# facebookresearch/momentum

Hardware: NVIDIA H100
Metric: GN iterations/sec (batched 72-joint IK) (higher is better)
Workload: dtype f32

## Files before the change

### include/momentum_b200.h

```cpp
#ifndef MOMENTUM_B200_H_
#define MOMENTUM_B200_H_

#include <stddef.h>
#include <stdint.h>

#ifdef __cplusplus
extern "C" {
#endif

#define MB2_PARAMETERS_PER_JOINT 7
#define MB2_MAX_MODEL_PARAMETERS 2048
#define MB2_PARAMETER_SET_WORDS 32

typedef enum mb2_status {
  MB2_OK = 0,
  MB2_ERR_INVALID_ARGUMENT = 1,
  MB2_ERR_CUDA = 2,
  MB2_ERR_UNSUPPORTED = 3
} mb2_status;

typedef enum mb2_instance_status {
  MB2_INSTANCE_OK = 0,
  MB2_INSTANCE_CHOLESKY_BREAKDOWN = 1,
  MB2_INSTANCE_NON_FINITE = 2
// ... 242 lines not shown
int mb2_solver_function_implicit_direction_device(mb2_solver_function* f, const float* parameters_device ,
                                                  const float* grad_parameters_device , float* direction_device ,
                                                  float* jacobian_direction_device , float* residual_device ,
                                                  float* gradient_rms_device , void* cuda_stream);

int mb2_solver_create(mb2_solver_function* f, const mb2_gauss_newton_options* opt, mb2_solver** out);
void mb2_solver_destroy(mb2_solver* s);
int mb2_solver_set_options(mb2_solver* s, const mb2_gauss_newton_options* opt);
int mb2_solver_set_enabled_parameters(mb2_solver* s, const uint64_t bits[MB2_PARAMETER_SET_WORDS]);
int mb2_solver_solve(mb2_solver* s, float* parameters, double* errors, int32_t* iterations, int32_t* status);
int mb2_solver_solve_async(mb2_solver* s, float* parameters);
int mb2_solver_wait(mb2_solver* s, double* errors, int32_t* iterations, int32_t* status);
int mb2_solver_solve_device(mb2_solver* s, float* parameters_device, void* cuda_stream);
int mb2_solver_get_results(mb2_solver* s, double* errors, int32_t* iterations, int32_t* status);
int mb2_solver_get_error_history(mb2_solver* s, double* history);
int mb2_solver_get_counters(mb2_solver* s, uint64_t* total_iterations, uint64_t* kernel_launches);
int mb2_solver_set_profiling(mb2_solver* s, int32_t enabled);
int mb2_solver_get_phase_times(mb2_solver* s, double ms[4], uint64_t launches[4]);
int mb2_solver_get_plan_stats(mb2_solver* s, int64_t stats[12]);
int mb2_solver_get_fused_profile(mb2_solver* s, int32_t* fused, int32_t* groups, double* kernel_ms, uint64_t phase_cycles[12]);
int mb2_solver_function_get_sweep_launch(mb2_solver_function* f, int32_t jacobian, int64_t out[5]);
int mb2_character_get_instance_launch(const mb2_character* c, int32_t op, int32_t backward, int32_t batch, int32_t num_points, int64_t out[6]);
int mb2_solver_function_get_input_gradient_launch(mb2_solver_function* f, int64_t out[6]);
int mb2_solver_get_solve_path(mb2_solver* s, int64_t out[15]);

typedef struct mb2_mixed_batch mb2_mixed_batch;
const char* mb2_mixed_batch_last_error(void);
int mb2_mixed_batch_create(int device, int32_t granule , mb2_mixed_batch** out);
void mb2_mixed_batch_destroy(mb2_mixed_batch* b);
int mb2_mixed_batch_add_rig(mb2_mixed_batch* b, const mb2_character* c, int32_t num_parameters, int32_t* rig_id);
int mb2_mixed_batch_use_limits(mb2_mixed_batch* b, int32_t enabled, float weight);
int mb2_mixed_batch_add_instance(mb2_mixed_batch* b, int32_t rig_id, int32_t num_constraints, const int32_t* parents, const float* offsets ,
                                 const float* weights , const float* targets , const float* theta0 , int32_t* instance_id);
int mb2_mixed_batch_set_parameters(mb2_mixed_batch* b, int32_t instance_id, const float* theta0);
int mb2_mixed_batch_solve(mb2_mixed_batch* b, const mb2_gauss_newton_options* opt);
int mb2_mixed_batch_get_result(mb2_mixed_batch* b, int32_t instance_id, float* theta, double* error, int32_t* iterations, int32_t* status);
int mb2_mixed_batch_get_results(mb2_mixed_batch* b, float* theta, const int64_t* theta_offsets, double* errors, int32_t* iterations, int32_t* status);
int mb2_mixed_batch_stats(mb2_mixed_batch* b, int64_t stats[6]);
int mb2_mixed_batch_bucket_info(mb2_mixed_batch* b, int32_t bucket, int64_t info[4]);

int mb2_character_clone(const mb2_character* c, int device, mb2_character** out);
int mb2_solver_function_clone(const mb2_solver_function* f, const mb2_character* c_on_device, int32_t batch, mb2_solver_function** out);
int mb2_character_device(const mb2_character* c);
const mb2_character* mb2_solver_function_character(const mb2_solver_function* f);
int32_t mb2_solver_function_num_error_functions(const mb2_solver_function* f);
int32_t mb2_solver_function_target_size(const mb2_solver_function* f, int32_t index);

// ... 17 lines not shown
```

### momentum_b200/csrc/ik_capi.cu

```cuda
#include "../../include/momentum_b200.h"

#include <cuda_runtime.h>
#include <nvtx3/nvToolsExt.h>

#include <algorithm>
#include <cfloat>
#include <cmath>
#include <cstdio>
#include <cstdlib>
#include <cstring>
#include <memory>
#include <string>
#include <vector>

#include "ik_chol_sched.h"
#include "ik_fused.cuh"
#include "ik_jtj_tc.cuh"
#include "ik_kernels.cuh"
#include "ik_plan.h"
#include "ik_solve_path.h"

using namespace mb2;

namespace {
// ... 163 lines not shown
  std::unique_ptr<DeviceSchedule> sched;
  SweepLaunch lastSweep[2]{};
  FunctionTables tables() const;
};

struct PhaseEvent {
  cudaEvent_t start, stop;
  int phase;
};

struct mb2_solver {
  mb2_solver_function* fn{nullptr};
  mb2_gauss_newton_options opt{};
  DeviceBuffer<float> dH, dDelta, dThetaOrig, dTheta0, dScale, dGradDotDelta, dThetaStage, dGrad, dTiles, dRadius, dRSaved;
  DeviceBuffer<double> dLastErrors, dTrialErrors, dHistory;
  DeviceBuffer<int32_t> dActive, dIterations, dStatus, dSearching, dActiveCount, dWorkCounter, dQrChunks;
  DeviceBuffer<unsigned long long> dPhaseCycles;
  DeviceBuffer<float> dPark;
  DeviceBuffer<uint32_t> dParkSlots;
  SolvePath path;
  cudaEvent_t fusedStart{nullptr}, fusedStop{nullptr};
  double fusedMs{0};
  int* hActiveCount{nullptr};
  char* hResults{nullptr};
  size_t hResultsBytes{0};
  bool resultsStaged{false};
  uint64_t totalIterations{0}, kernelLaunches{0};
  bool profiling{false};
  bool inKernelProfile{false};
  std::vector<PhaseEvent> events;
  double phaseMs[4]{0, 0, 0, 0};
  uint64_t phaseLaunches[4]{0, 0, 0, 0};
  size_t historyStride{0};
  ~mb2_solver() {
    if (hActiveCount) cudaFreeHost(hActiveCount);
    if (hResults) cudaFreeHost(hResults);
    if (fusedStart) cudaEventDestroy(fusedStart);
    if (fusedStop) cudaEventDestroy(fusedStop);
    for (auto& e : events) { cudaEventDestroy(e.start); cudaEventDestroy(e.stop); }
  }
};

CharacterTables mb2_character::tables() const {
  CharacterTables C{};
  C.numJoints = host.numJoints;
  C.numParams = host.numParams;
  C.parent = parent.p;
  C.offset = offset.p;
  C.prerot = prerot.p;
  C.ptOuter = ptOuter.p;
  C.ptInner = ptInner.p;
  C.ptVals = ptVals.p;
  C.ptOffsets = ptOffsets.p;
  C.numLevels = int(host.levelStart.size()) - 1;
  C.ptNnz = int(host.ptInner.size());
  C.levelStart = levelStart.p;
  C.levelJoints = levelJoints.p;
  return C;
}

SkeletonTables mb2_character::skeletonTables() const {
  return SkeletonTables{childStart.p, children.p,  ptColStart.p, ptColRows.p, ptColVals.p, invStart.p,
// ... 1406 lines not shown
  a.enabledList = f->dEnabledList.p;
  a.numEnabled = int(f->plan.enabledList.size());
  a.gradParameters = grad_parameters_device;
  a.direction = direction_device;
  a.jacobianDirection = jacobian_direction_device;
  a.residual = residual_device;
  a.gradientRms = gradient_rms_device;
  ImplicitDirectionConfig cfg;
  MB2_CUDA(implicitDirectionConfigure(a, cfg));
  MB2_CUDA(f->dJacobi.resize(std::max<size_t>(1, size_t(cfg.grid) * cfg.slotDoubles)));
  a.scratch = f->dJacobi.p;
  a.slotDoubles = cfg.slotDoubles;
  a.gramInShared = cfg.gramInShared ? 1 : 0;
  MB2_CUDA(launchImplicitDirection(a, cfg, st));
  return MB2_OK;
}

int mb2_solver_create(mb2_solver_function* f, const mb2_gauss_newton_options* opt, mb2_solver** out) {
  MB2_CHECK(f != nullptr && out != nullptr, "null argument");
  auto s = std::make_unique<mb2_solver>();
  s->fn = f;
  if (opt) s->opt = *opt; else mb2_default_gauss_newton_options(&s->opt);
  MB2_DEVICE_GUARD(f->ch->device);
  MB2_CUDA(cudaMallocHost(&s->hActiveCount, sizeof(int)));
  *out = s.release();
  return MB2_OK;
}
void mb2_solver_destroy(mb2_solver* s) { delete s; }
int mb2_solver_set_options(mb2_solver* s, const mb2_gauss_newton_options* opt) {
  MB2_CHECK(s != nullptr && opt != nullptr, "null argument");
  s->opt = *opt;
  return MB2_OK;
}
int mb2_solver_set_enabled_parameters(mb2_solver* s, const uint64_t* bits) {
  MB2_CHECK(s != nullptr, "null solver");
  return mb2_solver_function_set_enabled_parameters(s->fn, bits);
}
int mb2_solver_set_profiling(mb2_solver* s, int32_t enabled) {
  MB2_CHECK(s != nullptr, "null solver");
  s->profiling = enabled != 0;
  s->inKernelProfile = enabled >= 2;
  return MB2_OK;
}

namespace {
int planFigures(mb2_solver_function* f, int mode, bool schedDense, bool strips, PlanFigures& F, std::string& msg) {
  const int rc = ensurePlan(f, mode, schedDense, strips);
// ... 12 lines not shown
    F.gramCholValid = ds->gcValid;
    F.fusedBlobWords = ds->fLayout.words;
  }
  return MB2_OK;
}

}

int mb2_solver_solve_device(mb2_solver* s, float* theta, void* cudaStream) {
  MB2_CHECK(s != nullptr && theta != nullptr, "null argument");
  mb2_solver_function* f = s->fn;
  MB2_DEVICE_GUARD(f->ch->device);
  NvtxRange nvtxSolve("mb2::SolverT::solve");
  const mb2_gauss_newton_options& o = s->opt;
  const DeviceLimits lim = deviceLimits();
  std::string msg;
  const PlanFiguresFn plan = [f](int mode, bool schedDense, bool strips, PlanFigures& F, std::string& m) { return planFigures(f, mode, schedDense, strips, F, m); };
  int rc = chooseSolvePath(o, f->B, f->ch->host, f->host, plan, lim, s->path, msg);
  if (s->path.planMode != 0 && f->sched) f->sched->fusedGroups = s->path.fused.groups;
  if (rc != MB2_OK) {
    s->path = SolvePath{};
    return fail(rc, msg);
  }
  const SolvePath& P = s->path;
  cudaStream_t st = cudaStream ? (cudaStream_t)cudaStream : f->stream;
  const int B = f->B, n = f->ch->host.numParams;
  const int ns = f->plan.numCols;
  const int maxIt = int(std::min<uint64_t>(o.max_iterations, 1u << 30));
  const int minIt = int(std::min<uint64_t>(o.min_iterations, 1u << 30));
  MB2_CUDA(s->dIterations.resize(B));
  MB2_CUDA(s->dStatus.resize(B));
  if (o.store_error_history) {
    MB2_CUDA(s->dHistory.resize(size_t(B) * std::max(maxIt, 1)));
    MB2_CUDA(cudaMemsetAsync(s->dHistory.p, 0, size_t(B) * std::max(maxIt, 1) * sizeof(double), st));
    s->historyStride = size_t(std::max(maxIt, 1));
  }
  for (auto& e : s->events) { cudaEventDestroy(e.start); cudaEventDestroy(e.stop); }
  s->events.clear();
  if (s->profiling && (P.kind == kSolvePersistent || P.kind == kSolveGramCholesky)) {
    MB2_CUDA(s->dPhaseCycles.resize(16));
    MB2_CUDA(cudaMemsetAsync(s->dPhaseCycles.p, 0, 16 * sizeof(unsigned long long), st));
  }
  if (P.kind == kSolvePersistent) {
    const DeviceSchedule& ds = *f->sched;
    MB2_CUDA(s->dWorkCounter.resize(1));
    MB2_CUDA(cudaMemsetAsync(s->dWorkCounter.p, 0, sizeof(int32_t), st));
// ... 32 lines not shown
      MB2_CUDA(launchFusedSolve(fa, P.fused, lim.numSms, s->inKernelProfile, st));
    }
    if (s->profiling) MB2_CUDA(cudaEventRecord(s->fusedStop, st));
    s->kernelLaunches = 1;
    return MB2_OK;
  }
  const int ldH = roundUp(ns + 1, 16);
  const size_t hStride = size_t(ns + 1) * ldH;
  if (P.kind == kSolveDense || P.kind == kSolveTilesKMajor) MB2_CUDA(s->dH.resize(size_t(B) * hStride));
  const size_t tilesStride = P.strips ? size_t(f->sched->host.numTiles) * 256 + f->sched->host.nPad : 0;
  if (P.kind == kSolveTiles) MB2_CUDA(s->dTiles.resize(size_t(B) * tilesStride));
  const bool qr = P.kind == kSolveQr || P.kind == kSolveTrustRegionQr;
  if (qr) MB2_CUDA(s->dQrChunks.upload(P.qrChunkStarts, st));
  if (P.kind == kSolveTrustRegionQr) {
    MB2_CUDA(s->dRadius.upload(std::vector<float>(size_t(B), o.trust_region_radius), st));
    MB2_CUDA(s->dRSaved.resize(size_t(B) * P.trRSavedFloats));
  }
  const int ldG = cholGradientLd(ns);
  MB2_CUDA(s->dGrad.resize(size_t(B) * ldG));
  MB2_CUDA(s->dDelta.resize(size_t(B) * ns));
  MB2_CUDA(s->dTheta0.resize(size_t(B) * n));
  MB2_CUDA(s->dLastErrors.resize(B));
  MB2_CUDA(s->dActive.resize(B));
  MB2_CUDA(s->dActiveCount.resize(1));
  const bool lineSearch = o.do_line_search != 0 && P.kind != kSolveTrustRegionQr;
  if (lineSearch) {
    MB2_CUDA(s->dThetaOrig.resize(size_t(B) * n));
    MB2_CUDA(s->dTrialErrors.resize(B));
    MB2_CUDA(s->dScale.resize(B));
    MB2_CUDA(s->dSearching.resize(B));
    MB2_CUDA(s->dGradDotDelta.resize(B));
  }
  double* history = o.store_error_history ? s->dHistory.p : nullptr;

  const SweepArgs sweep = sweepArgs(f, theta, s->dActive.p);
  GramArgs g{};
  if (P.strips) {
    const DeviceSchedule& ds = *f->sched;
    g.batch = B;
    g.strips = f->dJ.p;
    g.stripStride = size_t(ds.gram.stride);
    g.residOff = ds.gram.residOff;
    g.active = s->dActive.p;
    g.numStrips = ds.gram.numStrips;
    g.numTiles = ds.host.numTiles;
    g.numTileCols = ds.host.numTileCols;
    g.nPad = ds.host.nPad;
// ... 74 lines not shown
    }
    gt.L = ds.gc.L;
    gt.tab = ds.gcTab.p;
  }
  CholArgs& step = qr ? t.q.c : (P.kind == kSolveGramCholesky ? gc.c : c);
  SweepArgs trial = sweepArgs(f, theta, s->dSearching.p);
  trial.errors = s->dTrialErrors.p;
  LineSearchArgs la{};
  la.batch = B; la.ns = ns; la.numParams = n; la.ldTheta = n;
  la.errors = f->dErrors.p;
  la.trialErrors = s->dTrialErrors.p;
  la.gradDotDelta = s->dGradDotDelta.p;
  la.scale = s->dScale.p;
  la.searching = s->dSearching.p;
  la.subsetVariant = o.subset_line_search;
  la.active = s->dActive.p;
  BookkeepingArgs ba{};
  ba.batch = B;
  ba.errors = f->dErrors.p; ba.lastErrors = s->dLastErrors.p; ba.active = s->dActive.p; ba.iterations = s->dIterations.p;
  ba.status = s->dStatus.p; ba.history = history;
  ba.theta = theta; ba.ldTheta = n; ba.numParams = n;
  ba.minIterations = minIt; ba.maxIterations = maxIt; ba.threshold = o.threshold; ba.activeCount = s->dActiveCount.p;

  s->kernelLaunches = 0;
  initSolveStateKernel<<<(B + 127) / 128, 128, 0, st>>>(B, s->dActive.p, s->dIterations.p, s->dStatus.p, s->dLastErrors.p, f->dErrors.p);
  MB2_CUDA(cudaGetLastError());
  MB2_CUDA(cudaMemcpyAsync(s->dTheta0.p, theta, size_t(B) * n * sizeof(float), cudaMemcpyDeviceToDevice, st));

  static const bool cholProfile = getenv("MB2_CHOL_PROFILE") != nullptr;
  constexpr int kPollEvery = 4;
  for (int it = 0; it < maxIt; ++it) {
    MB2_CUDA(cudaMemsetAsync(s->dActiveCount.p, 0, sizeof(int), st));
    recordPhaseStart(s, 0, st);
    MB2_CUDA(launchSweep(sweep, true, st, &f->lastSweep[1]));
    recordPhaseStop(s, st);
    step.iteration = it;
    step.profile = (it == 0 && cholProfile) ? 1 : 0;
    switch (P.kind) {
      case kSolveDense:
      case kSolveTilesKMajor:
      case kSolveTiles:
        recordPhaseStart(s, 1, st);
        if (P.kind == kSolveTiles) MB2_CUDA(launchGramTiles(g, P.gramThreads, st));
        else if ((rc = runJtJ(f, P.jtjMode, ns, c.H, ldH, hStride, s->dActive.p, st, s->dGrad.p, ldG)) != MB2_OK) return rc;
        recordPhaseStop(s, st);
        recordPhaseStart(s, 2, st);
        if (P.kind == kSolveDense) MB2_CUDA(launchCholesky(c, P.denseNb, P.denseInSmem, st));
        else MB2_CUDA(launchCholeskyScheduled(c, f->sched->dev, P.cholThreads, st));
        break;
      case kSolveGramCholesky:
        recordPhaseStart(s, 2, st);
        MB2_CUDA(launchGramCholesky(gc, f->sched->dev, f->sched->gcParams.get(), gt, s->inKernelProfile, st));
        break;
      case kSolveQr:
        recordPhaseStart(s, 2, st);
        MB2_CUDA(launchQrSolve(t.q, P.qrWidestChunk, st));
        break;
      default:
        recordPhaseStart(s, 2, st);
        MB2_CUDA(launchTrustRegionQr(t, st));
    }
    recordPhaseStop(s, st);
    if (lineSearch) {
      MB2_CUDA(cudaMemcpyAsync(s->dThetaOrig.p, theta, size_t(B) * n * sizeof(float), cudaMemcpyDeviceToDevice, st));
      initLineSearchKernel<<<(B + 127) / 128, 128, 0, st>>>(B, s->dActive.p, s->dSearching.p, s->dScale.p);
      MB2_CUDA(cudaGetLastError());
      for (int k = 0; k < 10; ++k) {
        MB2_CUDA(launchTrialUpdate(B, s->dThetaOrig.p, n, s->dDelta.p, ns, f->dDeviceCols.p, s->dScale.p, theta, s->dSearching.p, st));
        recordPhaseStart(s, 3, st);
        MB2_CUDA(launchSweep(trial, false, st, &f->lastSweep[0]));
        recordPhaseStop(s, st);
        la.step = k;
        MB2_CUDA(launchLineSearchStep(la, st));
        s->kernelLaunches += 2;
      }
      ba.iteration = it;
      MB2_CUDA(launchBookkeeping(ba, st));
      s->kernelLaunches += 1;
    }
    if (it + 1 < maxIt && it >= minIt && (it - minIt) % kPollEvery == kPollEvery - 1) {
      MB2_CUDA(cudaMemcpyAsync(s->hActiveCount, s->dActiveCount.p, sizeof(int), cudaMemcpyDeviceToHost, st));
      MB2_CUDA(cudaStreamSynchronize(st));
      if (*s->hActiveCount == 0) break;
    }
  }
  finalizeKernel<<<B, 128, 0, st>>>(B, n, theta, s->dTheta0.p, s->dStatus.p);
  MB2_CUDA(cudaGetLastError());
  s->kernelLaunches += 2;
  return MB2_OK;
}

static void collectProfile(mb2_solver* s) {
  if (s->profiling && s->path.kind == kSolvePersistent && s->fusedStart) {
    float ms = 0.f;
    s->fusedMs = cudaEventElapsedTime(&ms, s->fusedStart, s->fusedStop) == cudaSuccess ? double(ms) : 0.0;
  }
  if (s->profiling) {
    for (int k = 0; k < 4; ++k) { s->phaseMs[k] = 0; s->phaseLaunches[k] = 0; }
    for (auto& e : s->events) {
      float ms = 0.f;
      if (cudaEventElapsedTime(&ms, e.start, e.stop) == cudaSuccess) { s->phaseMs[e.phase] += ms; s->phaseLaunches[e.phase]++; }
    }
  }
}

int mb2_solver_get_results(mb2_solver* s, double* errors, int32_t* iterations, int32_t* status) {
  MB2_CHECK(s != nullptr, "null solver");
  mb2_solver_function* f = s->fn;
// ... 177 lines not shown
    a.T = c->tables();
    a.numChildren = int(c->host.children.size());
    a.batch = batch;
    a.P.numPoints = num_points;
    a.fromJointParameters = joint;
    MB2_CUDA(queryPositionsLaunch(a, backward != 0, &q));
  }
  instanceLaunchWords(q, out);
  return MB2_OK;
}

int mb2_solver_function_get_input_gradient_launch(mb2_solver_function* f, int64_t out[6]) {
  MB2_CHECK(f != nullptr && out != nullptr, "null argument");
  MB2_DEVICE_GUARD(f->ch->device);
  InputGradientArgs a{};
  a.T = f->tables();
  a.batch = f->B;
  InstanceLaunchQuery q;
  MB2_CUDA(launchInputGradients(a, nullptr, &q));
  instanceLaunchWords(q, out);
  return MB2_OK;
}

int mb2_solver_get_solve_path(mb2_solver* s, int64_t out[15]) {
  MB2_CHECK(s != nullptr && out != nullptr, "null argument");
  solvePathWords(s->path, out);
  return MB2_OK;
}

int mb2_solver_get_phase_times(mb2_solver* s, double ms[4], uint64_t launches[4]) {
  MB2_CHECK(s != nullptr, "null solver");
  for (int k = 0; k < 4; ++k) {
    if (ms) ms[k] = s->phaseMs[k];
    if (launches) launches[k] = s->phaseLaunches[k];
  }
  return MB2_OK;
}

}
```

### momentum_b200/csrc/ik_kernels.cu

```cuda
#include "ik_kernels.cuh"

#include <algorithm>
#include <cstdio>
#include <type_traits>

#include "ik_chol.cuh"
#include "ik_chol_sched.h"
#include "ik_jtj_tc.cuh"
#include "ik_ptx.cuh"
#include "ik_device.cuh"
#include "ik_jacobi.cuh"

namespace mb2 {

__device__ __forceinline__ double warpSum(double v) {
  for (int o = 16; o > 0; o >>= 1) v += __shfl_xor_sync(0xffffffffu, v, o);
  return v;
}

size_t sweepSmemPerInstance(const FunctionTables& T, int warpsPerInstance) {
  const size_t nPad = (T.numParams + 3) & ~3;
  const size_t jp = warpsPerInstance > 1 ? size_t((T.numJoints * kParametersPerJoint + 1) & ~1) : 0;
  return sizeof(float) * (nPad + jp + size_t((T.numJoints * kJointStateStride + 1) & ~1) + size_t((T.recStride + 1) & ~1) + 4 + 2 * size_t(warpsPerInstance));
}
// ... 69 lines not shown
    }
    g.sync();
  }
}

static int g_numSms = 0;
static int g_maxSmemOptin = 0;
static int g_maxSmemPerSm = 0;

cudaError_t launchSweep(const SweepArgs& a0, bool jacobian, cudaStream_t stream, SweepLaunch* out) {
  SweepArgs a = a0;
  if (out) *out = SweepLaunch{};
  const size_t budget = size_t(g_maxSmemOptin);
  const size_t per1 = sweepSmemPerInstance(a.T, 8);
  a.stageTables = (2 * per1 + sweepTableBytes(a.T, 1) + 16 <= budget) ? 1 : (2 * per1 + sweepTableBytes(a.T, 2) + 16 <= budget) ? 2 : 0;
  const size_t tableBytes = sweepTableBytes(a.T, a.stageTables) + 16;
  int groups = int((budget - tableBytes) / per1);
  if (groups < 1) return cudaErrorInvalidConfiguration;
  const int groupsOneWarp = int((budget - tableBytes) / sweepSmemPerInstance(a.T, 1));
  int W = 1;
  if (groupsOneWarp >= 16) {
    const int sms = std::max(g_numSms, 1);
    const int maxG = std::min(groupsOneWarp, kSweepMaxWarps), minG = std::min(12, maxG);
    long best = -1;
    if (a.batch < sms * minG) { groups = std::max(1, (a.batch + sms - 1) / sms); best = 0; }
    for (int gcand = maxG; gcand >= minG && best != 0; --gcand) {
      const long rounds = (a.batch + long(sms) * gcand - 1) / (long(sms) * gcand);
      if (best < 0 || rounds * gcand < best) { best = rounds * gcand; groups = gcand; }
    }
  } else {
    if (groups > 15) groups = 15;
    while (W < 8 && groups * W * 2 <= kSweepMaxWarps) W *= 2;
  }
  a.warpsPerInstance = W;
  const int warps = groups * W;
  const size_t per = sweepSmemPerInstance(a.T, W);
  const size_t smem = per * groups + tableBytes;
  if (smem > budget) return cudaErrorInvalidConfiguration;
  const int ctasNeeded = (a.batch + groups - 1) / groups;
  int ctasPerSm = (int)((size_t(g_maxSmemPerSm)) / (smem + 1024));
  if (ctasPerSm < 1) ctasPerSm = 1;
  if (ctasPerSm * warps > 32) ctasPerSm = 32 / warps > 0 ? 32 / warps : 1;
  int grid = g_numSms * ctasPerSm;
  if (grid > ctasNeeded) grid = ctasNeeded;
  if (grid < 1) grid = 1;
  if (out) *out = SweepLaunch{a.stageTables, W, groups, grid, int64_t(smem)};
  auto launch = [&](auto kernel) -> cudaError_t {
    const cudaError_t e = cudaFuncSetAttribute(kernel, cudaFuncAttributeMaxDynamicSharedMemorySize, int(smem));
    if (e != cudaSuccess) return e;
    kernel<<<grid, warps * 32, smem, stream>>>(a);
// ... 1903 lines not shown
  const uint64_t strides[2] = {uint64_t(fromGram ? 256 : a.ldH) * sizeof(float), uint64_t(fromGram ? a.tilesStride : a.hStride) * sizeof(float)};
  const uint32_t box[3] = {16u, 16u, 1u};
  e = makeTensorMap3d(&hmap, fromGram ? a.tilesIn : a.H, dims, strides, box, 64);
  if (e != cudaSuccess) return e;
  if (wide && prof) choleskyScheduledKernel<512, true><<<a.batch, 512, smem, stream>>>(hmap, a, sched);
  else if (wide) choleskyScheduledKernel<512, false><<<a.batch, 512, smem, stream>>>(hmap, a, sched);
  else if (prof) choleskyScheduledKernel<256, true><<<a.batch, 256, smem, stream>>>(hmap, a, sched);
  else choleskyScheduledKernel<256, false><<<a.batch, 256, smem, stream>>>(hmap, a, sched);
  return cudaGetLastError();
}

__device__ int acquireParkSlot(uint32_t* words, int numWords, int start) {
  for (int w = start % numWords;; w = (w + 1 == numWords) ? 0 : w + 1) {
    uint32_t freeBits = ~__ldcg(words + w);
    while (freeBits != 0u) {
      const int bit = __ffs(freeBits) - 1;
      if ((atomicOr(words + w, 1u << bit) & (1u << bit)) == 0u) return 32 * w + bit;
      freeBits &= freeBits - 1u;
    }
  }
}

template <bool kProfile, class Tables>
__global__ void __launch_bounds__(kGramThreads, 4) gramCholeskyKernel(const GramCholArgs a, const CholSchedDev S, const __grid_constant__ Tables P) {
  extern __shared__ __align__(16) float gcSmem[];
  const GramArgs& g = a.g;
  const CholArgs& c = a.c;
  const int b = blockIdx.x;
  if (c.active[b] == 0) return;
  const int n = c.ns, tid = threadIdx.x;
  const int warp = tid >> 5, lane = tid & 31, hw = tid >> 4, hl = tid & 15;
  constexpr int kWarps = kGramThreads / 32;
  float* U = gcSmem + (((128u - (smemAddr(gcSmem) & 127u)) & 127u) >> 2);
  const size_t tileFloats = size_t(S.numTiles) * 256, sweepFloats = g.stripStride + 64;
  const size_t uni = ((tileFloats > sweepFloats ? tileFloats : sweepFloats) + 3) & ~size_t(3);
  float* strips = U;
  float* resid = U + g.residOff;
  float* tiles = U;
  float* y = U + uni;
  float* gsub = y + S.nPad;
  int* flags = reinterpret_cast<int*>(gsub + ((n + 3) & ~3));
  unsigned long long* bar = reinterpret_cast<unsigned long long*>(flags + 4);
  const uint16_t* tab = P.tab;
  const GramCholLayout& L = P.L;
  long long pc[8] = {0, 0, 0, 0, 0, 0, 0, 0}, pt = 0;
  if constexpr (kProfile) pt = clock64();
#define MB2_GC(k) if constexpr (kProfile) { const long long now = clock64(); pc[k] += now - pt; pt = now; }
// ... 243 lines not shown
```

### momentum_b200/csrc/ik_kernels.cuh

```cuda
#pragma once

#include <cuda_runtime.h>

#include "ik_chol_sched.cuh"
#include "ik_chol_sched.h"
#include "ik_instance_launch.h"
#include "ik_solve_path.h"
#include "ik_types.h"

namespace mb2 {

struct SweepArgs {
  FunctionTables T;
  int32_t batch;
  const float* theta;
  int32_t ldTheta;
  const float* targets;
  const float* cweights;
  float* jacobian;
  double* errors;
  const int32_t* active;
  float* stateOut;
  int32_t stageTables;
  int32_t warpsPerInstance;
};

struct JtJArgs {
  int32_t batch;
  const float* jacobian;
  int32_t numCols, ldJ, kRows;
  int32_t ns;
  float* H;
  int32_t ldH;
  size_t hStride;
  const int32_t* active;
  float* g;
  int32_t ldG;
};

struct CholArgs {
  int32_t batch;
  float* H;
  size_t hStride;
  int32_t ns, ldH;
  float regularization;
// ... 290 lines not shown
```

### momentum_b200/csrc/ik_solve_path.cpp

```cpp
#include "ik_solve_path.h"

#include <algorithm>
#include <cstring>

#include "ik_chol.cuh"

namespace mb2 {

std::vector<int32_t> makeFusedBlob(const HostCharacter& h, const Plan& p, const std::vector<int32_t>& gramBlob, const std::vector<int32_t>& schedBlob, FusedBlobLayout& L) {
  std::vector<int32_t> blob;
  auto add = [&](const void* data, size_t bytes) {
    const int32_t off = int32_t(blob.size());
    const size_t words = (bytes + 3) / 4;
    blob.resize(blob.size() + words, 0);
    if (bytes) std::memcpy(blob.data() + off, data, bytes);
    while (blob.size() % 4) blob.push_back(0);
    return off;
  };
  L.parent = add(h.parent.data(), h.parent.size() * 4);
  L.offset = add(h.offset.data(), h.offset.size() * 4);
  L.prerot = add(h.prerot.data(), h.prerot.size() * 4);
  L.ptOuter = add(h.ptOuter.data(), h.ptOuter.size() * 4);
  L.ptInner = add(h.ptInner.data(), h.ptInner.size() * 4);
  L.ptVals = add(h.ptVals.data(), h.ptVals.size() * 4);
// ... 68 lines not shown
  const int sweep = P.stripStride + 64 + ((ch.numJoints * kJointStateStride + 3) & ~3) + ((ch.numJoints * kParametersPerJoint + 3) & ~3) + ((P.recStride + 3) & ~3);
  c.unionFloats = (std::max(P.numTiles * 256, sweep) + 3) & ~3;
  c.groupFloats = c.unionFloats + P.nPad + 2 * nc4 + np4 + 32;
  if (P.orderEntries / kGramWarps > kFusedMaxRounds) return c;
  const size_t fixed = 128 + size_t(P.fusedBlobWords) * 4 + 16;
  for (int g = kFusedMaxGroups; g >= 1; --g) {
    const size_t need = fixed + size_t(g) * c.groupFloats * sizeof(float);
    if (need <= size_t(maxSmemOptin)) {
      c.groups = g;
      c.smemBytes = need;
      break;
    }
  }
  return c;
}

int tileThreads(size_t smem, const DeviceLimits& lim) { return 2 * (smem + 1024) > size_t(lim.smemPerSm) ? 512 : 256; }

}

int chooseSolvePath(const mb2_gauss_newton_options& o, int batch, const HostCharacter& ch, const HostFunction& fn, const PlanFiguresFn& plan,
                    const DeviceLimits& lim, SolvePath& P, std::string& msg) {
  P = SolvePath{};
  auto refuse = [&](int code, const char* m) { msg = m; return code; };
  PlanFigures F;
  auto request = [&](int mode, bool schedDense, bool strips) {
    P.planMode = mode;
    P.schedDense = schedDense;
    P.strips = strips;
    const int rc = plan(mode, schedDense, strips, F, msg);
    P.fused = rc == MB2_OK && strips ? fusedConfigure(F, ch, lim.smemOptin) : FusedConfig{};
    return rc;
  };
  int cholMode = resolveCholeskyMode(o.cholesky_mode, fn.enabled);
  const bool useTr = o.linear_solver == MB2_LINEAR_SOLVER_TRUST_REGION_QR;
  const bool useQr = o.linear_solver == MB2_LINEAR_SOLVER_QR || useTr;
  if (useTr && !(o.trust_region_radius > 0.f)) return refuse(MB2_ERR_INVALID_ARGUMENT, "trust_region_radius must be positive");
  if (useQr) {
    if (o.jtj_mode == MB2_JTJ_SPARSE_TILES || o.cholesky_mode >= 2 || o.fused_mode >= MB2_FUSED_PERSISTENT)
      return refuse(MB2_ERR_UNSUPPORTED, "the QR step works on the dense Jacobian: it excludes the tile-sparse Gram, the tile Cholesky and the fused kernels");
    cholMode = 1;
  }
  bool useGram = cholMode >= 2 && (o.jtj_mode == MB2_JTJ_AUTO || o.jtj_mode == MB2_JTJ_SPARSE_TILES);
  if (o.jtj_mode == MB2_JTJ_SPARSE_TILES && cholMode < 2) return refuse(MB2_ERR_UNSUPPORTED, "MB2_JTJ_SPARSE_TILES needs the tile-scheduled Cholesky");
  int rc = request(cholMode >= 2 ? 2 : 1, cholMode == 2, useGram);
  if (rc != MB2_OK) return rc;
// ... 32 lines not shown
  if (P.jtjMode < 0) return refuse(MB2_ERR_UNSUPPORTED, "tensor-core JtJ does not support this shape");
  if (useQr) {
    int rows = qrMaxChunkRows(ns, size_t(200 * 1024));
    if (rows < 8) return refuse(MB2_ERR_UNSUPPORTED, "the QR step keeps R in shared memory: too many enabled parameters for this kernel");
    if (useTr) {
      rows = std::min(rows, std::max(8, ns / 2));
      if (trQrSmemFloats(ns, ch.numParams, ch.numJoints, rows) * sizeof(float) > size_t(220 * 1024))
        return refuse(MB2_ERR_UNSUPPORTED, "the trust-region QR kernel keeps R and the damping rows in shared memory: too many enabled parameters / joints");
      P.trRSavedFloats = (size_t(ns) * (ns + 1) / 2 + 3) & ~size_t(3);
    }
    P.qrMaxChunkRows = rows;
    P.qrChunkStarts.assign(1, 0);
    int r0 = 0, widest = 0;
    for (const auto& ef : fn.efs) {
      if (!(ef.weight > 0.f)) continue;
      const int size = jacobianBlockSize(ch, ef);
      for (int done = 0; done < size; done += rows) { const int p = std::min(rows, size - done); P.qrChunkStarts.push_back(r0 + done + p); widest = std::max(widest, p); }
      r0 += size;
    }
    P.qrWidestChunk = std::max(widest, 1);
    P.kind = useTr ? kSolveTrustRegionQr : kSolveQr;
  } else if (useGramChol) {
    P.kind = kSolveGramCholesky;
  } else if (useSchedule) {
    P.kind = useGram ? kSolveTiles : kSolveTilesKMajor;
    P.cholThreads = tileThreads(choleskyScheduledSmemBytes(ns, F.nPad, F.numTiles, F.schedBlobInts), lim);
    if (useGram) P.gramThreads = tileThreads(gramTilesSmemBytes(size_t(F.stripStride), F.gramBlobInts), lim);
  } else {
    P.kind = kSolveDense;
    const int eig = cholBlockSize(ns, 32);
    P.denseNb = eig <= 8 ? 8 : (eig <= 16 ? 16 : 32);
    P.denseInSmem = cholSmemBytes(ns, P.denseNb, true) <= size_t(lim.smemOptin);
  }
  return MB2_OK;
}

void solvePathWords(const SolvePath& p, int64_t out[kSolvePathWords]) {
  const int64_t w[kSolvePathWords] = {p.kind, p.planMode, p.schedDense, p.strips, p.jtjMode, p.denseNb, p.denseInSmem, p.gramThreads, p.cholThreads,
                                      p.qrMaxChunkRows, p.qrChunkStarts.empty() ? 0 : int64_t(p.qrChunkStarts.size()) - 1, p.qrWidestChunk,
                                      int64_t(p.trRSavedFloats), p.fused.groups, int64_t(p.fused.smemBytes)};
  std::copy(w, w + kSolvePathWords, out);
}

}
```

### momentum_b200/csrc/ik_solve_path.h

```cpp
#pragma once

#include <cstddef>
#include <cstdint>
#include <functional>
#include <string>
#include <vector>

#include "../../include/momentum_b200.h"
#include "ik_plan.h"

namespace mb2 {

constexpr int kFusedMaxGroups = 3;
constexpr int kFusedMaxRounds = 32;

struct FusedBlobLayout {
  int32_t parent, offset, prerot, ptOuter, ptInner, ptVals, ptOffsets, levelStart, levelJoints;
  int32_t efs, units, cells, contribs, limitData;
  int32_t cols;
  int32_t gram;
  int32_t sched;
  int32_t words;
};
std::vector<int32_t> makeFusedBlob(const HostCharacter& h, const Plan& p, const std::vector<int32_t>& gramBlob, const std::vector<int32_t>& schedBlob, FusedBlobLayout& L);
// ... 34 lines not shown
  kSolveNone = 0,
  kSolveDense = 1,
  kSolveTilesKMajor = 2,
  kSolveTiles = 3,
  kSolveGramCholesky = 4,
  kSolvePersistent = 5,
  kSolveQr = 6,
  kSolveTrustRegionQr = 7,
};

struct SolvePath {
  int32_t kind{kSolveNone};
  int32_t planMode{0};
  bool schedDense{false}, strips{false};
  int32_t jtjMode{0};
  int32_t denseNb{0};
  bool denseInSmem{false};
  int32_t gramThreads{0}, cholThreads{0};
  int32_t qrMaxChunkRows{0};
  std::vector<int32_t> qrChunkStarts;
  int32_t qrWidestChunk{0};
  size_t trRSavedFloats{0};
  FusedConfig fused;
};

int chooseSolvePath(const mb2_gauss_newton_options& o, int batch, const HostCharacter& ch, const HostFunction& fn, const PlanFiguresFn& plan,
                    const DeviceLimits& lim, SolvePath& out, std::string& msg);

constexpr int kSolvePathWords = 15;
void solvePathWords(const SolvePath& p, int64_t out[kSolvePathWords]);

}
```

### momentum_b200/solver.py

```python
from __future__ import annotations

import ctypes as C
import os
from dataclasses import dataclass
from typing import List, Optional, Sequence

import numpy as np

from . import character as mc

_HERE = os.path.dirname(os.path.abspath(__file__))
DEFAULT_LIB = os.path.join(_HERE, "lib", "libmomentum_b200.so")

SIZE_MAX = 2 ** 64 - 1

JTJ_AUTO, JTJ_FP32_SIMT, JTJ_TF32X3, JTJ_TF32, JTJ_SPARSE_TILES = 0, 1, 2, 3, 4
INSTANCE_OK, INSTANCE_CHOLESKY_BREAKDOWN, INSTANCE_NON_FINITE = 0, 1, 2
CHOLESKY_AUTO, CHOLESKY_DENSE_EIGEN, CHOLESKY_TILES_DENSE, CHOLESKY_TILES_SPARSE = 0, 1, 2, 3
FUSED_AUTO, FUSED_OFF, FUSED_PERSISTENT, FUSED_GRAM_CHOLESKY = 0, 1, 2, 3
FUSED_ON = FUSED_PERSISTENT
LINEAR_SOLVER_CHOLESKY, LINEAR_SOLVER_QR, LINEAR_SOLVER_TRUST_REGION_QR = 0, 1, 2


class MomentumB200Error(RuntimeError):
# ... 685 lines not shown

    def get_counters(self):
        a = C.c_uint64(0); b = C.c_uint64(0)
        self._check(self._L.mb2_solver_get_counters(self._h, C.byref(a), C.byref(b)))
        return a.value, b.value

    def get_plan_stats(self):
        st = (C.c_int64 * 12)()
        self._check(self._L.mb2_solver_get_plan_stats(self._h, st))
        keys = ["jacobian_nonzeros", "jacobian_columns", "ldj", "normal_parameters", "cholesky_tiles", "cholesky_tile_ops", "cholesky_levels", "rows",
                "strip_floats", "gram_macs", "gram_pairs", "fused_groups"]
        return dict(zip(keys, (int(v) for v in st)))

    FUSED_PHASES = ["fetch", "joint_parameters", "fk", "units", "cells", "gram", "parked_tiles", "chol_diag", "chol_panel", "chol_update",
                    "chol_backward", "update_bookkeeping"]

    def get_fused_profile(self):
        fused = C.c_int32(0); groups = C.c_int32(0); ms_ = C.c_double(0.0); cyc = (C.c_uint64 * 12)()
        self._check(self._L.mb2_solver_get_fused_profile(self._h, C.byref(fused), C.byref(groups), C.byref(ms_), cyc))
        return {"fused": int(fused.value), "groups": groups.value, "kernel_ms": ms_.value, "phase_cycles": dict(zip(self.FUSED_PHASES, (int(v) for v in cyc)))}

    SOLVE_PATH_KINDS = {0: None, 1: "dense", 2: "tiles_kmajor", 3: "tiles", 4: "gram_cholesky", 5: "persistent", 6: "qr", 7: "trust_region_qr"}
    SOLVE_PATH_KEYS = ["kind", "plan_mode", "sched_dense", "strips", "jtj_mode", "dense_nb", "dense_in_smem", "gram_threads", "chol_threads",
                       "qr_max_chunk_rows", "qr_chunks", "qr_widest_chunk", "tr_r_floats", "fused_groups", "fused_smem"]

    def get_solve_path(self) -> dict:
        out = (C.c_int64 * 15)()
        self._check(self._L.mb2_solver_get_solve_path(self._h, out))
        d = dict(zip(self.SOLVE_PATH_KEYS, (int(v) for v in out)))
        d["kind"] = self.SOLVE_PATH_KINDS[d["kind"]]
        return d

    def set_profiling(self, level):
        self._check(self._L.mb2_solver_set_profiling(self._h, int(level)))

    def get_phase_times(self):
        ms = (C.c_double * 4)(); ln = (C.c_uint64 * 4)()
        self._check(self._L.mb2_solver_get_phase_times(self._h, ms, ln))
        return list(ms), list(ln)


class MixedBatch(_Base):

    def __init__(self, device: int = 0, granule: int = 8, lib_path: Optional[str] = None):
        self._L = load_library(lib_path)
        self._h = C.c_void_p()
        self._check(self._L.mb2_mixed_batch_create(device, granule, C.byref(self._h)))
        self.device = device
        self._rigs: List[DeviceCharacter] = []
        self._sizes: List[int] = []
# ... 110 lines not shown
```

Before: 9.631 million.

## Split batch into two slices on separate streams to overlap sweep and Gram-Cholesky

For the Gram-Cholesky path without line search, and when the batch covers several waves of resident CTAs, the batch is split into two slices. Each slice runs its sweep and Gram-Cholesky kernels on its own stream, so one slice's sweep can overlap the other's factorization and fill idle SMs at phase boundaries. Streams are forked and joined with events around the periodic active-count poll, and each slice keeps its own active counter. The sweep launch plans its grid from the full batch so per-slice launches keep the same shape. This adds stream and event overhead, and slices can contend for SM resources.

```diff
diff --git a/include/momentum_b200.h b/include/momentum_b200.h
--- a/include/momentum_b200.h
+++ b/include/momentum_b200.h
@@ -288,7 +288,7 @@
 int mb2_solver_function_get_sweep_launch(mb2_solver_function* f, int32_t jacobian, int64_t out[5]);
 int mb2_character_get_instance_launch(const mb2_character* c, int32_t op, int32_t backward, int32_t batch, int32_t num_points, int64_t out[6]);
 int mb2_solver_function_get_input_gradient_launch(mb2_solver_function* f, int64_t out[6]);
-int mb2_solver_get_solve_path(mb2_solver* s, int64_t out[15]);
+int mb2_solver_get_solve_path(mb2_solver* s, int64_t out[16]);
 
 typedef struct mb2_mixed_batch mb2_mixed_batch;
 const char* mb2_mixed_batch_last_error(void);
diff --git a/momentum_b200/csrc/ik_capi.cu b/momentum_b200/csrc/ik_capi.cu
--- a/momentum_b200/csrc/ik_capi.cu
+++ b/momentum_b200/csrc/ik_capi.cu
@@ -209,6 +209,8 @@
   cudaEvent_t fusedStart{nullptr}, fusedStop{nullptr};
   double fusedMs{0};
   int* hActiveCount{nullptr};
+  cudaStream_t sliceStreams[kSolveSlices - 1]{};
+  cudaEvent_t forkEvent{nullptr}, joinEvents[kSolveSlices - 1]{};
   char* hResults{nullptr};
   size_t hResultsBytes{0};
   bool resultsStaged{false};
@@ -225,6 +227,11 @@
     if (fusedStart) cudaEventDestroy(fusedStart);
     if (fusedStop) cudaEventDestroy(fusedStop);
     for (auto& e : events) { cudaEventDestroy(e.start); cudaEventDestroy(e.stop); }
+    if (forkEvent) cudaEventDestroy(forkEvent);
+    for (int i = 0; i < kSolveSlices - 1; ++i) {
+      if (joinEvents[i]) cudaEventDestroy(joinEvents[i]);
+      if (sliceStreams[i]) cudaStreamDestroy(sliceStreams[i]);
+    }
   }
 };
 
@@ -1677,7 +1684,7 @@
   s->fn = f;
   if (opt) s->opt = *opt; else mb2_default_gauss_newton_options(&s->opt);
   MB2_DEVICE_GUARD(f->ch->device);
-  MB2_CUDA(cudaMallocHost(&s->hActiveCount, sizeof(int)));
+  MB2_CUDA(cudaMallocHost(&s->hActiveCount, kSolveSlices * sizeof(int)));
   *out = s.release();
   return MB2_OK;
 }
@@ -1736,6 +1743,7 @@
     s->path = SolvePath{};
     return fail(rc, msg);
   }
+  if (s->profiling) s->path.slices = 1;
   const SolvePath& P = s->path;
   cudaStream_t st = cudaStream ? (cudaStream_t)cudaStream : f->stream;
   const int B = f->B, n = f->ch->host.numParams;
@@ -1814,7 +1822,7 @@
   MB2_CUDA(s->dTheta0.resize(size_t(B) * n));
   MB2_CUDA(s->dLastErrors.resize(B));
   MB2_CUDA(s->dActive.resize(B));
-  MB2_CUDA(s->dActiveCount.resize(1));
+  MB2_CUDA(s->dActiveCount.resize(size_t(P.slices)));
   const bool lineSearch = o.do_line_search != 0 && P.kind != kSolveTrustRegionQr;
   if (lineSearch) {
     MB2_CUDA(s->dThetaOrig.resize(size_t(B) * n));
@@ -1935,45 +1943,104 @@
   ba.theta = theta; ba.ldTheta = n; ba.numParams = n;
   ba.minIterations = minIt; ba.maxIterations = maxIt; ba.threshold = o.threshold; ba.activeCount = s->dActiveCount.p;
 
+  const int S = P.slices;
+  auto sliceBegin = [&](int k) { return int(int64_t(B) * k / S); };
+  auto sliceStream = [&](int k) { return k == 0 ? st : s->sliceStreams[k - 1]; };
+  auto sliceSweep = [&](int k) {
+    const int b0 = sliceBegin(k);
+    SweepArgs a = sweep;
+    a.batch = sliceBegin(k + 1) - b0;
+    a.planBatch = B;
+    a.theta += size_t(b0) * a.ldTheta;
+    a.targets += size_t(b0) * a.T.targetStride;
+    if (a.T.weightsPerInstance) a.cweights += size_t(b0) * a.T.numWeights;
+    a.jacobian += size_t(b0) * a.T.jacobianStride;
+    a.errors += b0;
+    if (a.active) a.active += b0;
+    return a;
+  };
+  auto sliceGramCholesky = [&](int k) {
+    const int b0 = sliceBegin(k);
+    GramCholArgs a = gc;
+    a.g.batch = a.c.batch = sliceBegin(k + 1) - b0;
+    a.g.strips += size_t(b0) * a.g.stripStride;
+    a.g.active += b0;
+    CholArgs& c = a.c;
+    c.theta += size_t(b0) * c.ldTheta;
+    c.delta += size_t(b0) * c.ns;
+    c.errors += b0;
+    c.lastErrors += b0;
+    c.active += b0;
+    c.iterations += b0;
+    c.status += b0;
+    if (c.history) c.history += size_t(b0) * c.maxIterations;
+    c.activeCount += k;
+    return a;
+  };
+  if (S > 1 && !s->forkEvent) {
+    MB2_CUDA(cudaEventCreateWithFlags(&s->forkEvent, cudaEventDisableTiming));
+    for (int i = 0; i < kSolveSlices - 1; ++i) {
+      MB2_CUDA(cudaStreamCreateWithFlags(&s->sliceStreams[i], cudaStreamNonBlocking));
+      MB2_CUDA(cudaEventCreateWithFlags(&s->joinEvents[i], cudaEventDisableTiming));
+    }
+  }
+  auto fork = [&]() -> int {
+    if (S == 1) return MB2_OK;
+    MB2_CUDA(cudaEventRecord(s->forkEvent, st));
+    for (int k = 1; k < S; ++k) MB2_CUDA(cudaStreamWaitEvent(sliceStream(k), s->forkEvent, 0));
+    return MB2_OK;
+  };
+  auto join = [&]() -> int {
+    for (int k = 1; k < S; ++k) {
+      MB2_CUDA(cudaEventRecord(s->joinEvents[k - 1], sliceStream(k)));
+      MB2_CUDA(cudaStreamWaitEvent(st, s->joinEvents[k - 1], 0));
+    }
+    return MB2_OK;
+  };
+
   s->kernelLaunches = 0;
   initSolveStateKernel<<<(B + 127) / 128, 128, 0, st>>>(B, s->dActive.p, s->dIterations.p, s->dStatus.p, s->dLastErrors.p, f->dErrors.p);
   MB2_CUDA(cudaGetLastError());
   MB2_CUDA(cudaMemcpyAsync(s->dTheta0.p, theta, size_t(B) * n * sizeof(float), cudaMemcpyDeviceToDevice, st));
+  if ((rc = fork()) != MB2_OK) return rc;
 
   static const bool cholProfile = getenv("MB2_CHOL_PROFILE") != nullptr;
   constexpr int kPollEvery = 4;
   for (int it = 0; it < maxIt; ++it) {
-    MB2_CUDA(cudaMemsetAsync(s->dActiveCount.p, 0, sizeof(int), st));
-    recordPhaseStart(s, 0, st);
-    MB2_CUDA(launchSweep(sweep, true, st, &f->lastSweep[1]));
-    recordPhaseStop(s, st);
     step.iteration = it;
     step.profile = (it == 0 && cholProfile) ? 1 : 0;
-    switch (P.kind) {
-      case kSolveDense:
-      case kSolveTilesKMajor:
-      case kSolveTiles:
-        recordPhaseStart(s, 1, st);
-        if (P.kind == kSolveTiles) MB2_CUDA(launchGramTiles(g, P.gramThreads, st));
-        else if ((rc = runJtJ(f, P.jtjMode, ns, c.H, ldH, hStride, s->dActive.p, st, s->dGrad.p, ldG)) != MB2_OK) return rc;
-        recordPhaseStop(s, st);
-        recordPhaseStart(s, 2, st);
-        if (P.kind == kSolveDense) MB2_CUDA(launchCholesky(c, P.denseNb, P.denseInSmem, st));
-        else MB2_CUDA(launchCholeskyScheduled(c, f->sched->dev, P.cholThreads, st));
-        break;
-      case kSolveGramCholesky:
-        recordPhaseStart(s, 2, st);
-        MB2_CUDA(launchGramCholesky(gc, f->sched->dev, f->sched->gcParams.get(), gt, s->inKernelProfile, st));
-        break;
-      case kSolveQr:
-        recordPhaseStart(s, 2, st);
-        MB2_CUDA(launchQrSolve(t.q, P.qrWidestChunk, st));
-        break;
-      default:
-        recordPhaseStart(s, 2, st);
-        MB2_CUDA(launchTrustRegionQr(t, st));
+    for (int k = 0; k < S; ++k) {
+      const cudaStream_t sk = sliceStream(k);
+      MB2_CUDA(cudaMemsetAsync(s->dActiveCount.p + k, 0, sizeof(int), sk));
+      recordPhaseStart(s, 0, sk);
+      MB2_CUDA(launchSweep(sliceSweep(k), true, sk, &f->lastSweep[1]));
+      recordPhaseStop(s, sk);
+      switch (P.kind) {
+        case kSolveDense:
+        case kSolveTilesKMajor:
+        case kSolveTiles:
+          recordPhaseStart(s, 1, sk);
+          if (P.kind == kSolveTiles) MB2_CUDA(launchGramTiles(g, P.gramThreads, sk));
+          else if ((rc = runJtJ(f, P.jtjMode, ns, c.H, ldH, hStride, s->dActive.p, sk, s->dGrad.p, ldG)) != MB2_OK) return rc;
+          recordPhaseStop(s, sk);
+          recordPhaseStart(s, 2, sk);
+          if (P.kind == kSolveDense) MB2_CUDA(launchCholesky(c, P.denseNb, P.denseInSmem, sk));
+          else MB2_CUDA(launchCholeskyScheduled(c, f->sched->dev, P.cholThreads, sk));
+          break;
+        case kSolveGramCholesky:
+          recordPhaseStart(s, 2, sk);
+          MB2_CUDA(launchGramCholesky(sliceGramCholesky(k), f->sched->dev, f->sched->gcParams.get(), gt, s->inKernelProfile, sk));
+          break;
+        case kSolveQr:
+          recordPhaseStart(s, 2, sk);
+          MB2_CUDA(launchQrSolve(t.q, P.qrWidestChunk, sk));
+          break;
+        default:
+          recordPhaseStart(s, 2, sk);
+          MB2_CUDA(launchTrustRegionQr(t, sk));
+      }
+      recordPhaseStop(s, sk);
     }
-    recordPhaseStop(s, st);
     if (lineSearch) {
       MB2_CUDA(cudaMemcpyAsync(s->dThetaOrig.p, theta, size_t(B) * n * sizeof(float), cudaMemcpyDeviceToDevice, st));
       initLineSearchKernel<<<(B + 127) / 128, 128, 0, st>>>(B, s->dActive.p, s->dSearching.p, s->dScale.p);
@@ -1992,11 +2059,16 @@
       s->kernelLaunches += 1;
     }
     if (it + 1 < maxIt && it >= minIt && (it - minIt) % kPollEvery == kPollEvery - 1) {
-      MB2_CUDA(cudaMemcpyAsync(s->hActiveCount, s->dActiveCount.p, sizeof(int), cudaMemcpyDeviceToHost, st));
+      if ((rc = join()) != MB2_OK) return rc;
+      MB2_CUDA(cudaMemcpyAsync(s->hActiveCount, s->dActiveCount.p, size_t(S) * sizeof(int), cudaMemcpyDeviceToHost, st));
       MB2_CUDA(cudaStreamSynchronize(st));
-      if (*s->hActiveCount == 0) break;
+      int stillActive = 0;
+      for (int k = 0; k < S; ++k) stillActive += s->hActiveCount[k];
+      if (stillActive == 0) break;
+      if ((rc = fork()) != MB2_OK) return rc;
     }
   }
+  if ((rc = join()) != MB2_OK) return rc;
   finalizeKernel<<<B, 128, 0, st>>>(B, n, theta, s->dTheta0.p, s->dStatus.p);
   MB2_CUDA(cudaGetLastError());
   s->kernelLaunches += 2;
@@ -2220,7 +2292,7 @@
   return MB2_OK;
 }
 
-int mb2_solver_get_solve_path(mb2_solver* s, int64_t out[15]) {
+int mb2_solver_get_solve_path(mb2_solver* s, int64_t out[16]) {
   MB2_CHECK(s != nullptr && out != nullptr, "null argument");
   solvePathWords(s->path, out);
   return MB2_OK;
diff --git a/momentum_b200/csrc/ik_kernels.cu b/momentum_b200/csrc/ik_kernels.cu
--- a/momentum_b200/csrc/ik_kernels.cu
+++ b/momentum_b200/csrc/ik_kernels.cu
@@ -115,10 +115,11 @@
   if (groupsOneWarp >= 16) {
     const int sms = std::max(g_numSms, 1);
     const int maxG = std::min(groupsOneWarp, kSweepMaxWarps), minG = std::min(12, maxG);
+    const int planned = a.planBatch > 0 ? a.planBatch : a.batch;
     long best = -1;
-    if (a.batch < sms * minG) { groups = std::max(1, (a.batch + sms - 1) / sms); best = 0; }
+    if (planned < sms * minG) { groups = std::max(1, (planned + sms - 1) / sms); best = 0; }
     for (int gcand = maxG; gcand >= minG && best != 0; --gcand) {
-      const long rounds = (a.batch + long(sms) * gcand - 1) / (long(sms) * gcand);
+      const long rounds = (planned + long(sms) * gcand - 1) / (long(sms) * gcand);
       if (best < 0 || rounds * gcand < best) { best = rounds * gcand; groups = gcand; }
     }
   } else {
@@ -2068,7 +2069,7 @@
 }
 
 template <bool kProfile, class Tables>
-__global__ void __launch_bounds__(kGramThreads, 4) gramCholeskyKernel(const GramCholArgs a, const CholSchedDev S, const __grid_constant__ Tables P) {
+__global__ void __launch_bounds__(kGramThreads, kGramCholCtasPerSm) gramCholeskyKernel(const GramCholArgs a, const CholSchedDev S, const __grid_constant__ Tables P) {
   extern __shared__ __align__(16) float gcSmem[];
   const GramArgs& g = a.g;
   const CholArgs& c = a.c;
diff --git a/momentum_b200/csrc/ik_kernels.cuh b/momentum_b200/csrc/ik_kernels.cuh
--- a/momentum_b200/csrc/ik_kernels.cuh
+++ b/momentum_b200/csrc/ik_kernels.cuh
@@ -21,6 +21,7 @@
   double* errors;
   const int32_t* active;
   float* stateOut;
+  int32_t planBatch;
   int32_t stageTables;
   int32_t warpsPerInstance;
 };
diff --git a/momentum_b200/csrc/ik_solve_path.cpp b/momentum_b200/csrc/ik_solve_path.cpp
--- a/momentum_b200/csrc/ik_solve_path.cpp
+++ b/momentum_b200/csrc/ik_solve_path.cpp
@@ -114,6 +114,7 @@
 int chooseSolvePath(const mb2_gauss_newton_options& o, int batch, const HostCharacter& ch, const HostFunction& fn, const PlanFiguresFn& plan,
                     const DeviceLimits& lim, SolvePath& P, std::string& msg) {
   P = SolvePath{};
+  P.slices = 1;
   auto refuse = [&](int code, const char* m) { msg = m; return code; };
   PlanFigures F;
   auto request = [&](int mode, bool schedDense, bool strips) {
@@ -192,6 +193,9 @@
     P.kind = useTr ? kSolveTrustRegionQr : kSolveQr;
   } else if (useGramChol) {
     P.kind = kSolveGramCholesky;
+    const size_t perCta = gramCholeskySmemBytes(size_t(F.stripStride), ns, F.nPad, F.numTiles) + 1024;
+    const int resident = lim.numSms * std::min<int>(kGramCholCtasPerSm, int(size_t(lim.smemPerSm) / perCta));
+    if (o.do_line_search == 0 && resident > 0 && batch >= kSliceMinWaves * resident) P.slices = kSolveSlices;
   } else if (useSchedule) {
     P.kind = useGram ? kSolveTiles : kSolveTilesKMajor;
     P.cholThreads = tileThreads(choleskyScheduledSmemBytes(ns, F.nPad, F.numTiles, F.schedBlobInts), lim);
@@ -208,7 +212,7 @@
 void solvePathWords(const SolvePath& p, int64_t out[kSolvePathWords]) {
   const int64_t w[kSolvePathWords] = {p.kind, p.planMode, p.schedDense, p.strips, p.jtjMode, p.denseNb, p.denseInSmem, p.gramThreads, p.cholThreads,
                                       p.qrMaxChunkRows, p.qrChunkStarts.empty() ? 0 : int64_t(p.qrChunkStarts.size()) - 1, p.qrWidestChunk,
-                                      int64_t(p.trRSavedFloats), p.fused.groups, int64_t(p.fused.smemBytes)};
+                                      int64_t(p.trRSavedFloats), p.fused.groups, int64_t(p.fused.smemBytes), p.slices};
   std::copy(w, w + kSolvePathWords, out);
 }
 
diff --git a/momentum_b200/csrc/ik_solve_path.h b/momentum_b200/csrc/ik_solve_path.h
--- a/momentum_b200/csrc/ik_solve_path.h
+++ b/momentum_b200/csrc/ik_solve_path.h
@@ -80,12 +80,17 @@
   int32_t qrWidestChunk{0};
   size_t trRSavedFloats{0};
   FusedConfig fused;
+  int32_t slices{0};
 };
+
+constexpr int kGramCholCtasPerSm = 4;
+constexpr int kSolveSlices = 2;
+constexpr int kSliceMinWaves = 4;
 
 int chooseSolvePath(const mb2_gauss_newton_options& o, int batch, const HostCharacter& ch, const HostFunction& fn, const PlanFiguresFn& plan,
                     const DeviceLimits& lim, SolvePath& out, std::string& msg);
 
-constexpr int kSolvePathWords = 15;
+constexpr int kSolvePathWords = 16;
 void solvePathWords(const SolvePath& p, int64_t out[kSolvePathWords]);
 
 }
diff --git a/momentum_b200/solver.py b/momentum_b200/solver.py
--- a/momentum_b200/solver.py
+++ b/momentum_b200/solver.py
@@ -731,10 +731,10 @@
 
     SOLVE_PATH_KINDS = {0: None, 1: "dense", 2: "tiles_kmajor", 3: "tiles", 4: "gram_cholesky", 5: "persistent", 6: "qr", 7: "trust_region_qr"}
     SOLVE_PATH_KEYS = ["kind", "plan_mode", "sched_dense", "strips", "jtj_mode", "dense_nb", "dense_in_smem", "gram_threads", "chol_threads",
-                       "qr_max_chunk_rows", "qr_chunks", "qr_widest_chunk", "tr_r_floats", "fused_groups", "fused_smem"]
+                       "qr_max_chunk_rows", "qr_chunks", "qr_widest_chunk", "tr_r_floats", "fused_groups", "fused_smem", "slices"]
 
     def get_solve_path(self) -> dict:
-        out = (C.c_int64 * 15)()
+        out = (C.c_int64 * 16)()
         self._check(self._L.mb2_solver_get_solve_path(self._h, out))
         d = dict(zip(self.SOLVE_PATH_KEYS, (int(v) for v in out)))
         d["kind"] = self.SOLVE_PATH_KINDS[d["kind"]]
```

Measured after the change: 9.965 million, median of 6. +3.5%, better.
